# InSilicoModellingGroup/rdcFEs

Hardware: AMD Instinct MI355X
Metric: elements_assembled_per_sec (higher is better)
Workload: dtype f64; 1 GPU; PIHNA TET4 K(119): 10110954 tets, 1728000 nodes, 5 unknowns, params run/PIHNA/input.dat (shipped), order=lex, state of SURVEY App. C (background (0,0,0,7170,0) of the shipped field file, tumour values inside a sphere r = 0.25; see state_sensitivity); scatter=rowgather, kernel_variant=auto, parallelism=single GPU, rank0_local_elements=10110954, rank0_nnz=639395950

## Files before the change

### rdcfes_amd/csrc/rdc_prep.h

```cpp
#ifndef RDC_PREP_H
#define RDC_PREP_H
#include <stdint.h>
#include <string>
#include <vector>

namespace rdc {

struct HostPrep {
  int nen = 0, nvar = 0;
  int64_t n_elem = 0, n_node = 0, n_owned = 0;
  std::vector<int64_t> bptr;
  std::vector<int32_t> bcol;
  std::vector<uint16_t> eslot;
  int n_colours = 0;
  std::vector<int32_t> colour;
  std::vector<uint32_t> elem_order;
  std::vector<int64_t> colour_ptr;
  std::vector<uint64_t> first_mask;
  std::vector<uint8_t> first_rhs;
  bool rowgather_ok = false;
  int rg_block = 256;
  size_t rg_lds_bytes = 0;
  std::vector<uint32_t> pair_elem;
  std::vector<uint8_t> pair_local;
// ... 49 lines not shown

struct SolidGather {
  std::vector<uint32_t> gptr, gsrc;
  std::vector<int32_t> brow;
};
std::string solid_gather_build(const HostPrep& P, SolidGather& out);

struct HostPrepEv {
  static constexpr int MAXN = 16, NBP = 256, BLOCK = 256;
  struct Desc {
    uint32_t nown, nvis, ntouch, nb;
    uint32_t out_doubles;
    uint32_t min_node, max_node, pad;
  };
  struct Node {
    uint32_t bptr;
    uint16_t len, blk0;
    uint32_t obase;
    uint32_t node;
  };
  bool ok = false;
  int nls = 0;
  size_t max_out_doubles = 0;
  std::vector<Desc> desc;
  std::vector<uint32_t> nlist;
  std::vector<uint32_t> vloc;
  std::vector<uint32_t> vslot;
  std::vector<Node> ntab;
  std::vector<uint8_t> bpart;
  int64_t n_visits = 0, n_rows = 0;
  int64_t n_conflicts = 0;
  int64_t n_group_rows = 0;
  int64_t n_pass_instr = 0;
  static constexpr int PASS_COST_PIHNA[4] = {69, 54, 39, 24};
  static constexpr int PASS_COST_FLAT[4] = {40, 40, 40, 40};
  static constexpr int COLLISION_COST = 17;
};
std::string prep_build_ev(const HostPrep& P, const uint32_t* conn, size_t lds_budget_bytes, HostPrepEv& out, int64_t n_interior = -1);

#if defined(__HIPCC__)
#define RDC_EVL __host__ __device__ inline __attribute__((always_inline))
#else
#define RDC_EVL inline
#endif
namespace evl {
constexpr uint32_t IDLE = 0xFFFFFFFFu;
RDC_EVL uint32_t vloc_pack(const uint32_t (&pos)[4]) { return pos[0] | pos[1] << 8 | pos[2] << 16 | pos[3] << 24; }
RDC_EVL int vloc_pos(uint32_t pl, int j) { return (int)((pl >> (8 * j)) & 0xFF); }
RDC_EVL int vloc_rows(const int (&li)[4], int nown) { return (li[0] < nown) + (li[1] < nown) + (li[2] < nown) + (li[3] < nown); }
RDC_EVL void vslot_add(uint32_t (&sl)[2], int i, int j, uint32_t slot) { sl[i >> 1] |= (slot & 15u) << (16 * (i & 1) + 4 * j); }
RDC_EVL int vslot_get(uint32_t w0, uint32_t w1, int i, int j) { return (int)(((i < 2 ? w0 : w1) >> (16 * (i & 1) + 4 * j)) & 0xF); }
RDC_EVL int block(int a, int s) { return s * HostPrepEv::MAXN + a; }
RDC_EVL int block_node(int t) { return t & (HostPrepEv::MAXN - 1); }
RDC_EVL int block_slot(int t) { return t >> 4; }
RDC_EVL int seg_entry(int nv, int len, int a, int s, int b) { return a * (nv * len) + nv * s + b; }
RDC_EVL int seg_phase(uint32_t obase) { return (int)(obase & 1u); }
}

struct HostPrepCl {
  struct Limits { int max_nodes = 24, max_pairs = 192, max_elems = 64, max_row_doubles = 6000, pair_order = 1, img_per_block = 0; };
  struct Desc {
    uint16_t nown, npair, nelem, pad;
    uint32_t row_doubles;
    uint32_t min_node_max_node_pad;
  };
  struct Node {
// ... 75 lines not shown
```

### rdcfes_amd/csrc/rdc_prep_ev.cpp

```cpp
#include <algorithm>
#include <array>
#include <cstring>
#include <numeric>

#include "rdc_prep.h"

namespace rdc {

std::string prep_build_ev(const HostPrep& P, const uint32_t* conn, size_t lds_budget_bytes, HostPrepEv& E, int64_t n_interior) {
  E = HostPrepEv();
  if (P.nen != 4 || (P.nvar != 5 && P.nvar != 3)) return "element-visit lists exist for TET4 with 3 or 5 unknowns only";
  const size_t nv2 = (size_t)P.nvar * P.nvar;
  const int64_t n_elem = P.n_elem, n_node = P.n_node, n_owned = P.n_owned;
  if (n_owned <= 0) return "no owned nodes";
  if (P.bptr[(size_t)n_owned] >= ((int64_t)1 << 32)) return "more than 2^32 node blocks";
  constexpr int MAXN = HostPrepEv::MAXN, NBP = HostPrepEv::NBP, BLOCK = HostPrepEv::BLOCK;
  std::vector<int64_t> inc_ptr((size_t)n_node + 1, 0);
  for (int64_t x = 0; x < n_elem * 4; x++) inc_ptr[conn[x] + 1]++;
  for (int64_t n = 0; n < n_node; n++) inc_ptr[n + 1] += inc_ptr[n];
  std::vector<uint32_t> inc((size_t)inc_ptr[n_node]);
  {
    std::vector<int64_t> fill(inc_ptr.begin(), inc_ptr.end() - 1);
    for (int64_t e = 0; e < n_elem; e++)
      for (int i = 0; i < 4; i++) inc[fill[conn[e * 4 + i]]++] = (uint32_t)e;
  }
  const size_t budget_doubles = lds_budget_bytes / sizeof(double);
  std::vector<int32_t> cluster_of((size_t)n_owned, -1);
  std::vector<std::vector<uint32_t>> clusters;
  {
    std::vector<uint32_t> emark((size_t)n_elem, 0), nmark((size_t)n_node, 0), gain((size_t)n_owned, 0), gstamp((size_t)n_owned, 0);
    uint32_t stamp = 0;
    std::vector<uint32_t> cand, tmp, rejected;
    std::vector<int32_t> free_nb((size_t)n_owned, 0);
    int max_nb = 0;
    for (int64_t n = 0; n < n_owned; n++) {
      if (P.bptr[n + 1] - P.bptr[n] > NBP / MAXN) return "a node has more than 16 node blocks in its row (valence > 15): no element-visit lists";
      int c = 0;
      for (int64_t b = P.bptr[n]; b < P.bptr[n + 1]; b++) c += (P.bcol[b] != (int32_t)n && (int64_t)P.bcol[b] < n_owned);
// ... 97 lines not shown
#pragma omp parallel for schedule(dynamic, 256)
  for (int64_t w = 0; w < nwg; w++) {
    const std::vector<uint32_t>& cl = clusters[(size_t)w];
    std::vector<uint32_t>& vis = visits[(size_t)w];
    for (uint32_t n : cl)
      for (int64_t k = inc_ptr[n]; k < inc_ptr[n + 1]; k++) vis.push_back(inc[k]);
    std::sort(vis.begin(), vis.end());
    vis.erase(std::unique(vis.begin(), vis.end()), vis.end());
    std::vector<uint32_t>& t = touched[(size_t)w];
    for (uint32_t e : vis)
      for (int j = 0; j < 4; j++) t.push_back(conn[(int64_t)e * 4 + j]);
    std::sort(t.begin(), t.end());
    t.erase(std::unique(t.begin(), t.end()), t.end());
    std::vector<uint32_t> ordered(cl.begin(), cl.end());
    for (uint32_t m : t) if (!((int64_t)m < n_owned && cluster_of[m] == (int32_t)w)) ordered.push_back(m);
    t.swap(ordered);
    ntouch_w[(size_t)w] = (int32_t)t.size();
    if (t.size() > 255 || vis.size() > (size_t)BLOCK) {
#pragma omp atomic write
      fail = 1;
    }
  }
  if (fail) return "internal: cluster limits violated";
  int mx = 1;
  for (int64_t w = 0; w < nwg; w++) mx = std::max(mx, (int)ntouch_w[(size_t)w]);
  E.nls = (mx + 63) & ~63;
  E.nlist.assign((size_t)nwg * E.nls, 0);
  E.vloc.assign((size_t)nwg * BLOCK, 0xFFFFFFFFu);
  E.vslot.assign((size_t)nwg * BLOCK * 2, 0);
  E.ntab.assign((size_t)nwg * MAXN, HostPrepEv::Node{0, 0, 0, 0, 0});
  E.bpart.assign((size_t)nwg * NBP, 0);
  std::vector<int64_t> rows_w((size_t)nwg, 0), conf_w((size_t)nwg, 0), pass_w((size_t)nwg, 0), instr_w((size_t)nwg, 0);
  std::vector<size_t> img_w((size_t)nwg, 0);
#pragma omp parallel for schedule(dynamic, 256)
  for (int64_t w = 0; w < nwg; w++) {
    const std::vector<uint32_t>& cl = clusters[(size_t)w];
    const std::vector<uint32_t>& t = touched[(size_t)w];
    const std::vector<uint32_t>& vis = visits[(size_t)w];
    HostPrepEv::Desc& d = E.desc[(size_t)w];
    bool wfail = false;
    d.nown = (uint32_t)cl.size(); d.nvis = (uint32_t)vis.size(); d.ntouch = (uint32_t)t.size(); d.pad = 0;
    d.min_node = *std::min_element(cl.begin(), cl.end());
    d.max_node = *std::max_element(cl.begin(), cl.end());
    uint32_t* nl = &E.nlist[(size_t)w * E.nls];
    for (int x = 0; x < E.nls; x++) nl[x] = t[std::min<size_t>((size_t)x, t.size() - 1)];
    uint32_t blk = 0, ob = 0;
    for (size_t x = 0; x < cl.size(); x++) {
      const uint32_t n = cl[x];
      HostPrepEv::Node& nd = E.ntab[(size_t)w * MAXN + x];
      const int64_t len = P.bptr[n + 1] - P.bptr[n];
      nd.bptr = (uint32_t)P.bptr[n]; nd.len = (uint16_t)len; nd.blk0 = (uint16_t)x; nd.node = n;
      const uint32_t phase = (uint32_t)(((int64_t)nv2 * P.bptr[n]) & 1);
      if ((uint32_t)evl::seg_phase(ob) != phase) ob++;
      nd.obase = ob;
      ob += (uint32_t)(nv2 * (size_t)len);
      blk += (uint32_t)len;
      if (len > NBP / MAXN) wfail = true;
    }
    d.nb = blk;
    if (wfail) {
#pragma omp atomic write
      fail = 1;
      continue;
    }
    {
      uint8_t* bp = &E.bpart[(size_t)w * NBP];
// ... 179 lines not shown
        try_profile(prof, best_pl);
      }
    }
    if (!best_pl.ok) wfail = true;
    std::vector<int> fill_g(16, 0), maxr_g(16, 0);
    for (int x = 0; x < nlanes && !wfail; x++) {
      const V& v = vv[(size_t)x];
      const int best_g = best_pl.grp[(size_t)x];
      const int* pm = PERM4[PERM_R[v.r][(int)best_pl.q[(size_t)x]]];
      int perm[4];
      for (int i = 0; i < v.r; i++) perm[i] = v.own[pm[i]];
      for (int j = v.r; j < 4; j++) perm[j] = v.rest[j - v.r];
      maxr_g[best_g] = std::max(maxr_g[best_g], v.r);
      const size_t lane = (size_t)best_g * 16 + (size_t)fill_g[best_g]++;
      uint32_t li[4];
      for (int j = 0; j < 4; j++) {
        const uint32_t m = conn[(int64_t)v.e * 4 + perm[j]];
        li[j] = (uint32_t)(std::find(t.begin(), t.end(), m) - t.begin());
      }
      E.vloc[(size_t)w * BLOCK + lane] = evl::vloc_pack(li);
      rows_w[(size_t)w] += v.r;
      uint32_t sl2[2] = {0, 0};
      for (int i = 0; i < v.r; i++) {
        for (int j = 0; j < 4; j++) {
          const uint32_t sl = P.eslot[(size_t)v.e * 16 + (size_t)perm[i] * 4 + (size_t)perm[j]];
          if (sl > 15) wfail = true;
          evl::vslot_add(sl2, i, j, sl);
        }
        if (li[i] >= cl.size()) wfail = true;
      }
      E.vslot[((size_t)w * BLOCK + lane) * 2] = sl2[0];
      E.vslot[((size_t)w * BLOCK + lane) * 2 + 1] = sl2[1];
    }
    conf_w[(size_t)w] = best_pl.coll;
    instr_w[(size_t)w] = best_pl.instr;
    for (int g = 0; g < 16; g++) pass_w[(size_t)w] += maxr_g[g];
    if (wfail) {
#pragma omp atomic write
      fail = 1;
    }
  }
  if (fail) return "internal: element-visit list construction failed";
  for (int64_t w = 0; w < nwg; w++) {
    E.max_out_doubles = std::max(E.max_out_doubles, img_w[(size_t)w]);
    E.n_visits += (int64_t)E.desc[(size_t)w].nvis;
    E.n_rows += rows_w[(size_t)w];
    E.n_conflicts += conf_w[(size_t)w];
    E.n_group_rows += pass_w[(size_t)w];
    E.n_pass_instr += instr_w[(size_t)w];
  }
  E.ok = true;
  return std::string();
}

}
```

### rdcfes_amd/csrc/rdc_tet4_ev.h

```cpp
#ifndef RDC_TET4_EV_H
#define RDC_TET4_EV_H
#include "rdc_integrands.h"

namespace rdc {
namespace ev {

constexpr int NM = 16;
constexpr int NMG = 22;
constexpr int NBP = 256;
constexpr int MAXN = 16;
enum { M_E1, M_EoV, M_EPh, M_EQh, M_En, M_Ec, M_Eh, M_Ev, M_Ea, M_Ex, M_Ey, M_ETau, M_EdTc, M_Epv, M_Eg4, M_Edd,
       M_Xc, M_Yc, M_Zc, M_Xh, M_Yh, M_Zh };
constexpr bool symmetric_moment(int m) { return m != M_Epv; }
constexpr bool symmetric_moment_gen(int m) { return m != M_Epv && m != M_Edd && m != M_Xc && m != M_Yc && m != M_Xh && m != M_Yh; }

template <int EXP_MODE, class Sink, bool MIRROR = true, bool GEN = false>
RDC_HD void pihna_visit(const PihnaK& k, const double (&X)[4][3], const double (&U)[4][5], const int r, Sink& sink, const bool bg = false) {
  double e1[3], e2[3], e3[3];
#pragma unroll
  for (int d = 0; d < 3; d++) { e1[d] = X[1][d] - X[0][d]; e2[d] = X[2][d] - X[0][d]; e3[d] = X[3][d] - X[0][d]; }
  double g[4][3];
  g[1][0] = e2[1] * e3[2] - e2[2] * e3[1]; g[1][1] = e2[2] * e3[0] - e2[0] * e3[2]; g[1][2] = e2[0] * e3[1] - e2[1] * e3[0];
  g[2][0] = e3[1] * e1[2] - e3[2] * e1[1]; g[2][1] = e3[2] * e1[0] - e3[0] * e1[2]; g[2][2] = e3[0] * e1[1] - e3[1] * e1[0];
  g[3][0] = e1[1] * e2[2] - e1[2] * e2[1]; g[3][1] = e1[2] * e2[0] - e1[0] * e2[2]; g[3][2] = e1[0] * e2[1] - e1[1] * e2[0];
  const double det = e1[0] * g[1][0] + e1[1] * g[1][1] + e1[2] * g[1][2];
  const double inv = rcp(det), inv2 = inv * inv;
  const double adet = fabs(det);
#pragma unroll
  for (int d = 0; d < 3; d++) g[0][d] = -(g[1][d] + g[2][d] + g[3][d]);
  const double Wc = adet * (-2.0 / 15.0), Wh = adet * 0.075;
  const double a0 = Wc * (1.0 / 16.0), b36 = Wh * (1.0 / 36.0), w18 = Wh * (1.0 / 18.0);
  Pihna::Pt s[5];
  {
    double S[5];
#pragma unroll
    for (int v = 0; v < 5; v++) S[v] = (U[0][v] + U[1][v]) + (U[2][v] + U[3][v]);
#pragma unroll
    for (int q = 0; q < 5; q++) {
      double uq[5];
#pragma unroll
      for (int v = 0; v < 5; v++) uq[v] = (q == 0) ? 0.25 * S[v] : (S[v] * (1.0 / 6.0) + U[q == 0 ? 0 : q - 1][v] * (1.0 / 3.0));
      Pihna::point<EXP_MODE>(k, uq, nullptr, s[q]);
    }
  }
#define RDC_EV_SYM(m, beta)                                                                              \
  {                                                                                                      \
    const double Sm_ = a0 * beta[0] + b36 * ((beta[1] + beta[2]) + (beta[3] + beta[4]));                 \
    const double t_[4] = {w18 * beta[1], w18 * beta[2], w18 * beta[3], w18 * beta[4]};                   \
// ... 109 lines not shown
        RDC_EV_PT(b, ((sp == 1 ? s[q].c : s[q].h) > k.Lambda) ? (expr) : 0.0)                             \
        FSx = (scale) * (Wc * 0.25 * b[0] + Wh * (1.0 / 6.0) * ((b[1] + b[2]) + (b[3] + b[4])));         \
        _Pragma("unroll") for (int j = 0; j < 4; j++) fx[j] = (scale) * (Wh * (1.0 / 3.0)) * b[j + 1];   \
      }
      RDC_EV_F(FS1, f1, Td, s[q].dT)
      RDC_EV_F(FS2, f2, Tt, s[q].dT * (sp == 1 ? s[q].c : s[q].h))
      RDC_EV_F(FS3, f3, Tt, s[q].Tau)
#undef RDC_EV_F
      {
        RDC_EV_PT(b, ((sp == 1 ? s[q].c : s[q].h) > k.Lambda) ? s[q].Tau : 0.0)
        sD = Td * (Wc * b[0] + Wh * ((b[1] + b[2]) + (b[3] + b[4])));
      }
      {
        RDC_EV_PT(b, ((sp == 1 ? s[q].c : s[q].h) > k.Lambda) ? s[q].Tau * (sp == 1 ? s[q].c : s[q].h) : 0.0)
        sZ = Tt * (Wc * b[0] + Wh * ((b[1] + b[2]) + (b[3] + b[4])));
      }
      const int mX = sp == 1 ? M_Xc : M_Xh, mY = sp == 1 ? M_Yc : M_Yh, mZ = sp == 1 ? M_Zc : M_Zh;
#pragma unroll
      for (int i = 0; i < 4; i++) if (i < r) {
        const double gko = go[0] * g[i][0] + go[1] * g[i][1] + go[2] * g[i][2];
        const double gkv = gv[0] * g[i][0] + gv[1] * g[i][1] + gv[2] * g[i][2];
        const double xb = gko * FS1 + gkv * FS2, yb = gkv * FS3;
#pragma unroll
        for (int j = 0; j < 4; j++) {
          const double dd_ = g[i][0] * g[j][0] + g[i][1] * g[j][1] + g[i][2] * g[j][2];
          sink.mom(mX, i, j, xb + gko * f1[j] + gkv * f2[j]);
          sink.mom(mY, i, j, yb + gkv * f3[j] + sD * dd_);
          if (!MIRROR || j >= i) sink.mom(mZ, i, j, sZ * dd_);
        }
        sink.rhs(sp, i, -(sD * gko + sZ * gkv));
      }
    }
  }
  if (!bg) {
    RDC_EV_PT(oneVe, 1.0 - s[q].Ve)
    RDC_EV_PT(Pq, s[q].Ve * s[q].rV)
    RDC_EV_PT(Qq, oneVe[q] * s[q].rV)
    RDC_EV_SYM(M_EoV, oneVe)
    {
      RDC_EV_PT(Ph, Pq[q] * s[q].h)
      RDC_EV_SYM(M_EPh, Ph)
      RDC_EV_PT(xx, k.Tc2h * (Pq[q] * s[q].c) + k.Th2c * Ph[q])
      RDC_EV_SYM(M_Ex, xx)
    }
    {
      RDC_EV_PT(Qh, Qq[q] * s[q].h)
      RDC_EV_SYM(M_EQh, Qh)
      RDC_EV_PT(yy, k.Tc2h * (Qq[q] * s[q].c) + k.Th2c * Qh[q])
      RDC_EV_SYM(M_Ey, yy)
    }
    {
      RDC_EV_PT(G, s[q].n + k.Tn_c * (s[q].c * s[q].n) + k.Tn_h * (s[q].h * s[q].n) + k.Tn_v * (s[q].v * s[q].n) + k.Th2n * (oneVe[q] * s[q].h))
      RDC_EV_RHS(0, G)
    }
    {
      RDC_EV_PT(G, s[q].c + k.Tprod_c * (s[q].Tau * s[q].c) - k.Tc2h * (oneVe[q] * s[q].c) + k.Th2c * (s[q].h - oneVe[q] * s[q].h) - k.Tn_c * (s[q].c * s[q].n))
      RDC_EV_RHS(1, G)
    }
    {
      RDC_EV_PT(G, s[q].h + k.Tc2h * (oneVe[q] * s[q].c) - k.Th2c * (s[q].h - oneVe[q] * s[q].h) - k.Tn_h * (s[q].h * s[q].n) - k.Th2n * (oneVe[q] * s[q].h))
      RDC_EV_RHS(2, G)
    }
  }
  if (!bg) {
    RDC_EV_PT(G, s[q].a + k.Tsec_c * s[q].c + k.Tsec_h * s[q].h - k.Tupt * (s[q].v * s[q].a) - k.Tdec * s[q].a)
    RDC_EV_RHS(4, G)
  }
#undef RDC_EV_RHS
  {
    const double one[5] = {1.0, 1.0, 1.0, 1.0, 1.0};
    RDC_EV_SYM(M_E1, one)
  }
  if (!bg) {
    { RDC_EV_PT(b, s[q].n) RDC_EV_SYM(M_En, b) }
    { RDC_EV_PT(b, s[q].c) RDC_EV_SYM(M_Ec, b) }
    { RDC_EV_PT(b, s[q].h) RDC_EV_SYM(M_Eh, b) }
    { RDC_EV_PT(b, s[q].dT * s[q].c) RDC_EV_SYM(M_EdTc, b) }
  }
  { RDC_EV_PT(b, s[q].v) RDC_EV_SYM(M_Ev, b) }
  if (k.Tupt != 0.0) { RDC_EV_PT(b, s[q].a) RDC_EV_SYM(M_Ea, b) }
  { RDC_EV_PT(b, s[q].Tau) RDC_EV_SYM(M_ETau, b) }
#undef RDC_EV_SYM
#undef RDC_EV_PT
}

RDC_HD bool pihna_background(const double (&U)[4][5]) {
  bool b = true;
#pragma unroll
  for (int j = 0; j < 4; j++) b = b && U[j][0] == 0.0 && U[j][1] == 0.0 && U[j][2] == 0.0 && U[j][4] == 0.0 && U[j][3] > 0.0;
  return b;
}

template <int NMT>
RDC_HD void pihna_expand(const PihnaK& k, const double (&e)[NMT], double (&o)[25]) {
  const double E1 = e[M_E1], EoV = e[M_EoV], EPh = e[M_EPh], EQh = e[M_EQh], En = e[M_En], Ec = e[M_Ec], Eh = e[M_Eh], Ev = e[M_Ev];
  const double x = e[M_Ex], y = e[M_Ey], pcj = k.Tprod_c * e[M_EdTc], pv = e[M_Epv];
  o[0] = E1 - k.Tn_c * Ec - k.Tn_h * Eh - k.Tn_v * Ev;
  o[1] = -(k.Tn_c * En + k.Th2n * EPh);
  o[2] = -(k.Tn_h * En + k.Th2n * EPh + k.Th2n * EoV);
  o[3] = k.Th2n * EQh - k.Tn_v * En;
  o[4] = 0.0;
  o[5] = k.Tn_c * Ec - pcj;
  o[6] = E1 - k.Tprod_c * e[M_ETau] - pcj + k.Tc2h * EoV + x + k.Tn_c * En;
  o[7] = x - pcj - k.Th2c * (E1 - EoV);
  o[8] = -(pcj + y);
// ... 28 lines not shown
```

### rdcfes_amd/csrc/rdc_tet4_ev.hip

```cpp
#include "rdc_internal.h"
#include <type_traits>
#include "rdc_tet4_ev.h"
#include "rdc_ev_phases.h"

namespace rdc {

template <int ABL_>
struct EvSink {
  static constexpr int ABL = ABL_ == 4 ? 0 : ABL_;
  double* p[4][4];
  double* pr[4];
  double sum = 0.0;
  __device__ __forceinline__ void mom(int m, int i, int j, double v) {
    if (ABL == 0) __hip_atomic_fetch_add(p[i][j] + m * ev::NBP, v, __ATOMIC_RELAXED, __HIP_MEMORY_SCOPE_WORKGROUP);
    else if (ABL == 1) p[i][j][m * ev::NBP] = v;
    else sum += v;
  }
  __device__ __forceinline__ void rhs(int a, int i, double v) {
    if (ABL == 0) __hip_atomic_fetch_add(pr[i] + a * ev::MAXN, v, __ATOMIC_RELAXED, __HIP_MEMORY_SCOPE_WORKGROUP);
    else if (ABL == 1) pr[i][a * ev::MAXN] = v;
    else sum += v;
  }
};


namespace {
template <bool GEN, int NM>
__device__ __forceinline__ void ev_read_moments(const double* lds, const int blk, const int mirror, double (&e)[NM]) {
  constexpr auto sym = [](const int m) { return GEN ? ev::symmetric_moment_gen(m) : ev::symmetric_moment(m); };
  constexpr int NS = [=]() { int n = 0; for (int m = 0; m < NM; m++) n += sym(m); return n; }();
#pragma unroll
  for (int m = 0; m < NM; m++) e[m] = lds[m * ev::NBP + blk];
  if (mirror != blk) {
    double t[NS];
#pragma unroll
    for (int m = 0, x = 0; m < NM; m++)
      if (sym(m)) t[x++] = lds[m * ev::NBP + mirror];
    evl::lds_batch();
    evl::lds_land(t);
#pragma unroll
    for (int m = 0, x = 0; m < NM; m++)
      if (sym(m)) e[m] += t[x++];
  }
}
}

template <int EXP_MODE, int MINW, int ABL = 0, bool GEN = false, int NROW = 5>
__global__ void __launch_bounds__(256, MINW)
k_tet4_ev(const HostPrepEv::Desc* __restrict__ desc, const uint32_t* __restrict__ nlist, const uint32_t* __restrict__ vloc,
          const uint32_t* __restrict__ vslot, const HostPrepEv::Node* __restrict__ ntab, const uint8_t* __restrict__ bpart,
          const uint32_t* __restrict__ wg_perm, const PihnaK k, const double* __restrict__ rec, double* __restrict__ val,
          double* __restrict__ rhs, const int nls, const int wg_begin, const int xcd_n, const int stagger,
          long long* __restrict__ stamps, const int bg_skip) {
  static_assert(NROW == 4 || NROW == 5, "all five equation rows, or all but the a row");
  constexpr int BLOCK = 256, NP = 4;
  constexpr bool TL = ABL == 4;
  long long ts[11];
#define RDC_TS(x) if (TL) ts[x] = __builtin_amdgcn_s_memtime()
  RDC_TS(0);
  constexpr int NM = GEN ? ev::NMG : ev::NM, NBP = ev::NBP, MAXN = ev::MAXN;
  extern __shared__ __attribute__((aligned(16))) double lds[];
  __shared__ __attribute__((aligned(16))) HostPrepEv::Node snode[MAXN];
  typedef __attribute__((address_space(3))) void* lds_ptr;
  typedef const __attribute__((address_space(1))) void* glb_ptr;
  if (stagger > 0 && blockIdx.x < 1024u) {
    const unsigned lds_base = __builtin_amdgcn_s_getreg((7 << 11) | 6);
    const uint32_t slot = lds_base == 0 ? 0u : (lds_base < 144u ? 1u : 2u);
    for (uint32_t i = 0; i < slot * (uint32_t)stagger; i++) __builtin_amdgcn_s_sleep(16);
  }
  int wl = (int)blockIdx.x;
  if (xcd_n > 0) {
    const int q = xcd_n >> 3, rem = xcd_n & 7, x = wl & 7;
    wl = x * q + (x < rem ? x : rem) + (wl >> 3);
  }
  int w = wl + wg_begin;
  if (wg_perm) w = (int)wg_perm[w];
  const int tid = threadIdx.x, lane = tid & 63, wv = tid >> 6;
  double* const R = lds + NM * NBP;
  double* const recs = R + 5 * MAXN;
  evl::zero_slice<NM * NBP * 8>(lds, __builtin_amdgcn_readfirstlane(wv));
  if (tid < 5 * MAXN) lds[NM * NBP + tid] = 0.0;
  const int rounds = nls >> 6;
  uint32_t nid = 0;
  if (wv < rounds) nid = nlist[(size_t)w * nls + wv * 64 + lane];
  const uint32_t pl = vloc[(size_t)w * BLOCK + tid];
  const uint2 sl = reinterpret_cast<const uint2*>(vslot)[(size_t)w * BLOCK + tid];
  const HostPrepEv::Desc d = desc[w];
  const int mirror = (int)bpart[(size_t)w * NBP + tid];
  if (tid < MAXN) snode[tid] = ntab[(size_t)w * MAXN + tid];
  if (wv < rounds) {
    const char* src = reinterpret_cast<const char*>(rec) + (size_t)nid * (NP * 16);
#pragma unroll
    for (int p = 0; p < NP; p++)
      __builtin_amdgcn_global_load_lds((glb_ptr)(src + p * 16), (lds_ptr)evl::rec_at(recs, nls, p, wv * 64), 16, 0, 0);
  }
  RDC_TS(1);
  asm volatile("s_waitcnt vmcnt(0)" ::: "memory");
  RDC_TS(2);
  __syncthreads();
  RDC_TS(3);
  if (pl != evl::IDLE) {
    double X[4][3], U[4][5];
    int li[4];
#pragma unroll
    for (int j = 0; j < 4; j++) {
      li[j] = evl::vloc_pos(pl, j);
      double rr[2 * NP];
#pragma unroll
      for (int p = 0; p < NP; p++) {
        const double2 v2 = evl::rec_piece(recs, nls, p, li[j]);
        rr[2 * p] = v2.x; rr[2 * p + 1] = v2.y;
      }
      X[j][0] = rr[0]; X[j][1] = rr[1]; X[j][2] = rr[2];
#pragma unroll
      for (int v = 0; v < 5; v++) U[j][v] = rr[3 + v];
    }
    const int r = evl::vloc_rows(li, (int)d.nown);
    EvSink<ABL> sink;
    evl::aim(sink, lds, R, li, r, sl);
    const bool bg = bg_skip && __builtin_amdgcn_ballot_w64(!ev::pihna_background(U)) == 0;
    if (ABL != 3) ev::pihna_visit<EXP_MODE, EvSink<ABL>, true, GEN>(k, X, U, r, sink, bg);
    if (ABL == 2 && sink.sum == 1.2345e300) rhs[0] = sink.sum;
  }
  if (TL) asm volatile("s_waitcnt lgkmcnt(0)" ::: "memory");
  RDC_TS(4);
  __syncthreads();
  RDC_TS(5);
  double e[NM];
  const int bn = evl::block_node(tid), bs = evl::block_slot(tid);
  const bool has = bn < (int)d.nown && bs < (int)snode[bn < (int)d.nown ? bn : 0].len;
  if (has) ev_read_moments<GEN>(lds, tid, mirror, e);
  if (tid < (int)d.nown * 5) {
    const int n = tid / 5, a = tid - n * 5;
    rhs[(size_t)snode[n].node * 5 + a] = R[a * MAXN + n];
  }
  RDC_TS(6);
  __syncthreads();
  if (has) {
    double o[25];
    ev::pihna_expand(k, e, o);
    const int len = (int)snode[bn].len;
    double* dst = lds + snode[bn].obase + evl::seg_entry(5, len, 0, bs, 0);
#pragma unroll
    for (int a = 0; a < NROW; a++)
#pragma unroll
      for (int b = 0; b < 5; b++) dst[evl::seg_entry(5, len, a, 0, b)] = o[a * 5 + b];
  }
  RDC_TS(7);
  __syncthreads();
  RDC_TS(8);
  {
    const int wvu = __builtin_amdgcn_readfirstlane(wv);
    HostPrepEv::Node nd[4];
    evl::wave_nodes(snode, wvu, nd);
    const HostPrepEv::Node nd01[2] = {nd[0], nd[1]}, nd23[2] = {nd[2], nd[3]};
    const bool on01[2] = {wvu < (int)d.nown, wvu + 4 < (int)d.nown}, on23[2] = {wvu + 8 < (int)d.nown, wvu + 12 < (int)d.nown};
    if (on01[0]) evl::store_segments<25, 2, 5 * NROW>(lds, val, nd01, on01, lane);
    if (on23[0]) evl::store_segments<25, 2, 5 * NROW>(lds, val, nd23, on23, lane);
  }
  if (TL) {
    RDC_TS(9);
    if (stagger == 0) asm volatile("s_waitcnt vmcnt(0)" ::: "memory");
    RDC_TS(10);
    if (lane == 0 && stamps) {
// ... 3 lines not shown
      o[11] = (long long)__builtin_amdgcn_s_getreg((31 << 11) | 4) | ((long long)__builtin_amdgcn_s_getreg((31 << 11) | 20) << 32);
    }
  }
#undef RDC_TS
}


namespace {
__device__ __forceinline__ void evl_dma16(const void* g, const void* lds_base) {
  const uint32_t b = __builtin_amdgcn_readfirstlane((uint32_t)(uintptr_t)lds_base);
  asm volatile("s_mov_b32 m0, %1\n\ts_nop 0\n\tglobal_load_lds_dwordx4 %0, off" ::"v"(g), "s"(b) : "memory", "m0");
}
}
namespace {
struct EvqLists {
  static constexpr int PL = 0, SL = 1024, MISC = SL + 2048, MIRROR = MISC, SNODE = MISC + 256, DESC = MISC + 512, NL = MISC + 544;
  static constexpr int bytes(int nls) { return NL + 2 * nls * 4; }
};
}
template <int EXP_MODE, bool TL, bool GEN = false, int NROW = 5>
__global__ void __launch_bounds__(256, GEN ? 2 : 3)
k_tet4_evq(const HostPrepEv::Desc* __restrict__ desc, const uint32_t* __restrict__ nlist, const uint32_t* __restrict__ vloc,
           const uint32_t* __restrict__ vslot, const HostPrepEv::Node* __restrict__ ntab, const uint8_t* __restrict__ bpart,
           const PihnaK k, const double* __restrict__ rec, double* __restrict__ val, double* __restrict__ rhs, const int nls,
           const int wg_begin, const int wg_count, long long* __restrict__ stamps, const int bg_skip, int* __restrict__ ticket,
           const uint32_t* __restrict__ wg_perm) {
  static_assert(NROW == 4 || NROW == 5, "k_tet4_ev");
  constexpr int BLOCK = 256, NP = 4;
  constexpr int NM = GEN ? ev::NMG : ev::NM, NBP = ev::NBP, MAXN = ev::MAXN;
  extern __shared__ __attribute__((aligned(16))) double lds[];
  __shared__ __attribute__((aligned(16))) HostPrepEv::Node snode[MAXN];
  __shared__ uint8_t smirror[NBP];
  __shared__ int s_nown;
  __shared__ int s_tk[2];
  double* const R = lds + NM * NBP;
  double* const recs = R + 5 * MAXN;
  char* const lists = reinterpret_cast<char*>(recs + (size_t)NP * nls * 2);
  const int rounds = nls >> 6;
  auto lds_barrier = [&]() { asm volatile("s_waitcnt lgkmcnt(0)\n\ts_barrier" ::: "memory"); };
  const int wv = __builtin_amdgcn_readfirstlane((int)(threadIdx.x >> 6));
  constexpr int NONE = 0x7fffffff;
  int c0 = (int)blockIdx.x, c1 = c0 + (int)gridDim.x, c2 = c0 + 2 * (int)gridDim.x;
  auto cluster_of = [&](const int c) -> int { return c < wg_count ? (wg_perm ? (int)wg_perm[wg_begin + c] : wg_begin + c) : -1; };
  int w0c = cluster_of(c0), w1c = cluster_of(c1), w2c = cluster_of(c2);
#define RDC_TS(x) if (TL && stamps && c0 < wg_count && lane == 0) stamps[((int64_t)c0 * 4 + wv) * 12 + x] = __builtin_amdgcn_s_memtime()
  auto fetch = [&](const int w, const uint32_t nid, const int w2, const int nb2, const int lane) {
    if (wv < rounds) {
      const char* src = reinterpret_cast<const char*>(rec) + (size_t)nid * (NP * 16);
#pragma unroll
      for (int p = 0; p < NP; p++) evl_dma16(src + p * 16, evl::rec_at(recs, nls, p, wv * 64));
    }
    if (wv == 0) evl_dma16(reinterpret_cast<const char*>(vloc + (size_t)w * BLOCK) + lane * 16, lists + EvqLists::PL);
    else if (wv < 3) evl_dma16(reinterpret_cast<const char*>(vslot + (size_t)w * BLOCK * 2) + (wv - 1) * 1024 + lane * 16, lists + EvqLists::SL + (wv - 1) * 1024);
    else {
      if (lane < 34) {
        const char* src = lane < 16 ? reinterpret_cast<const char*>(bpart + (size_t)w * NBP) + lane * 16
                        : lane < 32 ? reinterpret_cast<const char*>(ntab + (size_t)w * MAXN) + (lane - 16) * 16
                                    : reinterpret_cast<const char*>(desc + w) + (lane - 32) * 16;
        evl_dma16(src, lists + EvqLists::MISC);
      }
      if (w2 >= 0 && lane < (nls >> 2)) evl_dma16(reinterpret_cast<const char*>(nlist + (size_t)w2 * nls) + lane * 16, lists + EvqLists::NL + nb2 * nls * 4);
    }
  };
  {
    uint32_t nid0 = 0;
    if (wv < rounds) nid0 = nlist[(size_t)w0c * nls + threadIdx.x];
    asm volatile("s_waitcnt vmcnt(0)" : "+v"(nid0)::"memory");
    fetch(w0c, nid0, w1c, 1, (int)(threadIdx.x & 63));
  }
  int tk = NONE;
  bool pending = false;
#pragma unroll 1
  for (int it = 0;; it++) {
    int lane;
    asm volatile("v_mbcnt_lo_u32_b32 %0, -1, 0\n\tv_mbcnt_hi_u32_b32 %0, -1, %0" : "=v"(lane));
    RDC_TS(0);
    evl::zero_slice<NM * NBP * 8>(lds, wv);
    if (wv * 64 + lane < 5 * MAXN) lds[NM * NBP + wv * 64 + lane] = 0.0;
    asm volatile("s_waitcnt vmcnt(0)" : "+v"(tk)::"memory");
    if (pending && wv == 0 && lane == 0) s_tk[0] = tk == NONE ? NONE : 3 * (int)gridDim.x + tk;
    RDC_TS(1);
    lds_barrier();
    RDC_TS(2);
    if (pending) { c2 = __builtin_amdgcn_readfirstlane(s_tk[0]); w2c = cluster_of(c2); }
    if (c0 >= wg_count) break;
    {
      const int tid = wv * 64 + lane;
      const uint32_t pl = *reinterpret_cast<const uint32_t*>(lists + EvqLists::PL + tid * 4);
      const uint2 sl = *reinterpret_cast<const uint2*>(lists + EvqLists::SL + tid * 8);
      const int nown = (int)reinterpret_cast<const HostPrepEv::Desc*>(lists + EvqLists::DESC)->nown;
      {
        const int blk = evl::block(((wv >> 1) << 3) | (lane & 7), ((wv & 1) << 3) | (lane >> 3));
        smirror[blk] = *reinterpret_cast<const uint8_t*>(lists + EvqLists::MIRROR + blk);
        if (tid < MAXN) snode[tid] = *reinterpret_cast<const HostPrepEv::Node*>(lists + EvqLists::SNODE + tid * 16);
        if (tid == 0) s_nown = nown;
      }
      if (pl != evl::IDLE) {
        double X[4][3], U[4][5];
        int li[4];
#pragma unroll
        for (int j = 0; j < 4; j++) {
          li[j] = evl::vloc_pos(pl, j);
          double rr[2 * NP];
#pragma unroll
          for (int p = 0; p < NP; p++) {
            const double2 v2 = evl::rec_piece(recs, nls, p, li[j]);
            rr[2 * p] = v2.x; rr[2 * p + 1] = v2.y;
          }
          X[j][0] = rr[0]; X[j][1] = rr[1]; X[j][2] = rr[2];
#pragma unroll
          for (int v = 0; v < 5; v++) U[j][v] = rr[3 + v];
        }
        const int r = evl::vloc_rows(li, nown);
        EvSink<0> sink;
        evl::aim(sink, lds, R, li, r, sl);
        const bool bg = bg_skip && __builtin_amdgcn_ballot_w64(!ev::pihna_background(U)) == 0;
        ev::pihna_visit<EXP_MODE, EvSink<0>, true, GEN>(k, X, U, r, sink, bg);
      }
    }
    RDC_TS(3);
    lds_barrier();
    RDC_TS(4);
    asm volatile("v_mbcnt_lo_u32_b32 %0, -1, 0\n\tv_mbcnt_hi_u32_b32 %0, -1, %0" : "=v"(lane));
    const int bn = ((wv >> 1) << 3) | (lane & 7), bs = ((wv & 1) << 3) | (lane >> 3), blk = evl::block(bn, bs);
    int nown = s_nown, mirror = (int)smirror[blk];
    uint32_t bn_len = reinterpret_cast<const uint32_t*>(snode + bn)[1], bn_obase = snode[bn].obase;
    uint32_t base8 = snode[8].obase;
    uint32_t nid = 0;
    if (c1 < wg_count && wv < rounds) nid = *reinterpret_cast<const uint32_t*>(lists + EvqLists::NL + (((it + 1) & 1) * nls + wv * 64 + lane) * 4);
    evl::lds_batch();
    evl::lds_land(nown, mirror); evl::lds_land(bn_len, bn_obase); evl::lds_land(base8, nid);
    nown = __builtin_amdgcn_readfirstlane(nown);
    base8 = __builtin_amdgcn_readfirstlane(base8);
    bn_len &= 0xFFFFu;
    if (c1 < wg_count) fetch(w1c, nid, w2c, it & 1, lane);
    tk = NONE;
    if (c2 < wg_count && wv == 0 && lane == 0) {
      const int one = 1;
      asm volatile("global_atomic_add %0, %1, %2, off sc0" : "=v"(tk) : "v"(ticket), "v"(one) : "memory");
    }
    pending = true;
    double e[NM];
    const bool has = bn < nown && bs < (int)bn_len;
#pragma unroll
    for (int m = 0; m < NM; m++) e[m] = 0.0;
    if (has) ev_read_moments<GEN>(lds, blk, mirror, e);
    {
      const int tid = wv * 64 + lane;
      if (tid < nown * 5) {
        const int n = tid / 5, a = tid - n * 5;
        rhs[(size_t)snode[n].node * 5 + a] = R[a * MAXN + n];
      }
    }
    double o[25];
    ev::pihna_expand(k, e, o);
    lds_barrier();
#pragma unroll 1
    for (int h = 0; h < 2; h++) {
      const int n0 = h * 8;
      if (n0 >= nown) break;
      const uint32_t base = h == 0 ? 0u : (base8 & ~1u);
      if ((wv >> 1) == h && has) {
        const int len = (int)bn_len;
        double* dst = lds + (bn_obase - base) + evl::seg_entry(5, len, 0, bs, 0);
#pragma unroll
        for (int a = 0; a < NROW; a++)
#pragma unroll
          for (int b = 0; b < 5; b++) dst[evl::seg_entry(5, len, a, 0, b)] = o[a * 5 + b];
      }
      evl::v4u_t raw[2];
      evl::wave_nodes_read(snode, n0 + wv, raw);
      HostPrepEv::Node ndh[2];
      evl::wave_nodes_land(raw, ndh);
      lds_barrier();
      const int n1 = nown < n0 + 8 ? nown : n0 + 8;
      const bool on[2] = {n0 + wv < n1, n0 + wv + 4 < n1};
      if (on[0]) evl::store_segments<25, 2, 5 * NROW>(lds, val, ndh, on, lane, base);
      lds_barrier();
    }
// ... 66 lines not shown
```

Measured before the change: 7.488 billion elements/s.

## Skip dead moment LDS reads for all-background clusters and remap record slots

Each wave writes a per-wave background flag to LDS. When all four waves in a cluster visited only background elements, the moment read stage loads only the moments a background visit can produce and zeros the rest. This cuts LDS reads and mirror adds. Host prep also adds an LDS bank-conflict model and reassigns non-owned record slots (a remap of vloc and nlist) to reduce conflicts on 128-bit record reads. The cost is extra branching and templated read variants, and the remap changes ntouch and could mis-map slots if it is wrong.

```diff
diff --git a/rdcfes_amd/csrc/rdc_lds_model.h b/rdcfes_amd/csrc/rdc_lds_model.h
--- /dev/null
+++ b/rdcfes_amd/csrc/rdc_lds_model.h
@@ -0,0 +1,117 @@
+#ifndef RDC_LDS_MODEL_H
+#define RDC_LDS_MODEL_H
+#include <cstdint>
+
+#include "rdc_prep.h"
+
+namespace rdc {
+namespace ldsm {
+
+inline int group_b128(const int lane) {
+  const int l = lane & 31;
+  const bool first = l < 4 || (l >= 12 && l < 16) || (l >= 20 && l < 28);
+  return 2 * (lane >> 5) + (first ? 0 : 1);
+}
+inline int group_b64(const int lane) { return lane >> 4; }
+
+inline int group_cycles(const uint32_t* addr, const int n, const int width) {
+  uint32_t seen[16][16];
+  int cnt[16] = {0};
+  int worst = 0;
+  for (int x = 0; x < n; x++) {
+    const int s = (int)((addr[x] / (uint32_t)width) & 15u);
+    bool dup = false;
+    for (int y = 0; y < cnt[s] && !dup; y++) dup = seen[s][y] == addr[x];
+    if (!dup && cnt[s] < 16) seen[s][cnt[s]++] = addr[x];
+    if (cnt[s] > worst) worst = cnt[s];
+  }
+  return worst;
+}
+
+struct Cycles {
+  int64_t ideal = 0, cycles = 0;
+  Cycles& operator+=(const Cycles& o) { ideal += o.ideal; cycles += o.cycles; return *this; }
+};
+
+template <class Group>
+inline Cycles wave_cycles(const uint32_t (&addr)[64], const bool (&active)[64], const int width, Group group) {
+  uint32_t a[4][16];
+  int n[4] = {0, 0, 0, 0};
+  for (int lane = 0; lane < 64; lane++)
+    if (active[lane]) { const int g = group(lane); if (n[g] < 16) a[g][n[g]++] = addr[lane]; }
+  Cycles c;
+  for (int g = 0; g < 4; g++) { c.ideal += n[g] > 0; c.cycles += group_cycles(a[g], n[g], width); }
+  return c;
+}
+
+
+inline Cycles record_reads(const uint32_t* vloc, const int pieces, const uint8_t* remap = nullptr) {
+  Cycles c;
+  for (int wv = 0; wv < 4; wv++)
+    for (int j = 0; j < 4; j++) {
+      uint32_t addr[64];
+      bool active[64];
+      for (int lane = 0; lane < 64; lane++) {
+        const uint32_t pl = vloc[wv * 64 + lane];
+        active[lane] = pl != evl::IDLE;
+        const int pos = evl::vloc_pos(pl, j);
+        addr[lane] = active[lane] ? 16u * (uint32_t)(remap ? remap[pos] : pos) : 0u;
+      }
+      const Cycles one = wave_cycles(addr, active, 16, group_b128);
+      c.ideal += pieces * one.ideal;
+      c.cycles += pieces * one.cycles;
+    }
+  return c;
+}
+
+enum Mapping { MAP_EV = 0, MAP_EVQ = 1 };
+inline int lane_block(const Mapping map, const int wv, const int lane) {
+  if (map == MAP_EV) return wv * 64 + lane;
+  return evl::block(((wv >> 1) << 3) | (lane & 7), ((wv & 1) << 3) | (lane >> 3));
+}
+inline bool lane_has(const HostPrepEv::Desc& d, const HostPrepEv::Node* ntab, const int blk) {
+  const int bn = evl::block_node(blk), bs = evl::block_slot(blk);
+  return bn < (int)d.nown && bs < (int)ntab[bn].len;
+}
+
+inline void moment_reads(const HostPrepEv::Desc& d, const HostPrepEv::Node* ntab, const uint8_t* bpart, const Mapping map, Cycles& own, Cycles& mirror) {
+  for (int wv = 0; wv < 4; wv++) {
+    uint32_t a_own[64], a_mir[64];
+    bool on_own[64], on_mir[64];
+    for (int lane = 0; lane < 64; lane++) {
+      const int blk = lane_block(map, wv, lane);
+      on_own[lane] = lane_has(d, ntab, blk);
+      on_mir[lane] = on_own[lane] && (int)bpart[blk] != blk;
+      a_own[lane] = 8u * (uint32_t)blk;
+      a_mir[lane] = 8u * (uint32_t)bpart[blk];
+    }
+    own += wave_cycles(a_own, on_own, 8, group_b64);
+    mirror += wave_cycles(a_mir, on_mir, 8, group_b64);
+  }
+}
+
+inline Cycles image_writes(const HostPrepEv::Desc& d, const HostPrepEv::Node* ntab, const Mapping map, const int nrow) {
+  Cycles c;
+  const uint32_t base8 = d.nown > 8 ? (ntab[8].obase & ~1u) : 0u;
+  for (int wv = 0; wv < 4; wv++)
+    for (int a = 0; a < nrow; a++)
+      for (int b = 0; b < 5; b++) {
+        uint32_t addr[64];
+        bool active[64];
+        for (int lane = 0; lane < 64; lane++) {
+          const int blk = lane_block(map, wv, lane);
+          active[lane] = lane_has(d, ntab, blk);
+          addr[lane] = 0;
+          if (!active[lane]) continue;
+          const HostPrepEv::Node& nd = ntab[evl::block_node(blk)];
+          const uint32_t base = map == MAP_EVQ && evl::block_node(blk) >= 8 ? base8 : 0u;
+          addr[lane] = 8u * (nd.obase - base + (uint32_t)evl::seg_entry(5, (int)nd.len, a, evl::block_slot(blk), b));
+        }
+        c += wave_cycles(addr, active, 8, group_b64);
+      }
+  return c;
+}
+
+}
+}
+#endif
diff --git a/rdcfes_amd/csrc/rdc_prep.h b/rdcfes_amd/csrc/rdc_prep.h
--- a/rdcfes_amd/csrc/rdc_prep.h
+++ b/rdcfes_amd/csrc/rdc_prep.h
@@ -105,6 +105,9 @@
   int64_t n_conflicts = 0;
   int64_t n_group_rows = 0;
   int64_t n_pass_instr = 0;
+  int64_t lds_rec_ideal = 0, lds_rec = 0, lds_rec_identity = 0;
+  struct LdsExpansion { int64_t own_ideal = 0, own = 0, mirror_ideal = 0, mirror = 0, image_ideal = 0, image = 0; };
+  LdsExpansion lds_exp[2];
   static constexpr int PASS_COST_PIHNA[4] = {69, 54, 39, 24};
   static constexpr int PASS_COST_FLAT[4] = {40, 40, 40, 40};
   static constexpr int COLLISION_COST = 17;
diff --git a/rdcfes_amd/csrc/rdc_prep_ev.cpp b/rdcfes_amd/csrc/rdc_prep_ev.cpp
--- a/rdcfes_amd/csrc/rdc_prep_ev.cpp
+++ b/rdcfes_amd/csrc/rdc_prep_ev.cpp
@@ -4,6 +4,7 @@
 #include <numeric>
 
 #include "rdc_prep.h"
+#include "rdc_lds_model.h"
 
 namespace rdc {
 
@@ -167,6 +168,7 @@
   E.bpart.assign((size_t)nwg * NBP, 0);
   std::vector<int64_t> rows_w((size_t)nwg, 0), conf_w((size_t)nwg, 0), pass_w((size_t)nwg, 0), instr_w((size_t)nwg, 0);
   std::vector<size_t> img_w((size_t)nwg, 0);
+  std::vector<int64_t> rec_w((size_t)nwg, 0), rec_ident_w((size_t)nwg, 0), rec_ideal_w((size_t)nwg, 0), mom_w((size_t)nwg * 12, 0);
 #pragma omp parallel for schedule(dynamic, 256)
   for (int64_t w = 0; w < nwg; w++) {
     const std::vector<uint32_t>& cl = clusters[(size_t)w];
@@ -412,6 +414,97 @@
       E.vslot[((size_t)w * BLOCK + lane) * 2] = sl2[0];
       E.vslot[((size_t)w * BLOCK + lane) * 2 + 1] = sl2[1];
     }
+    if (!wfail) {
+      const int nown = (int)cl.size(), ntouch = (int)t.size(), limit = std::min(E.nls, 255);
+      uint32_t* vl = &E.vloc[(size_t)w * BLOCK];
+      std::array<std::array<uint8_t, 16>, 64> cnt;
+      for (auto& c : cnt) c.fill(0);
+      std::vector<std::vector<uint8_t>> occ((size_t)ntouch);
+      for (int lane = 0; lane < BLOCK; lane++) {
+        if (vl[lane] == evl::IDLE) continue;
+        for (int j = 0; j < 4; j++) {
+          const int g = ((lane >> 6) * 4 + j) * 4 + ldsm::group_b128(lane & 63);
+          std::vector<uint8_t>& o = occ[(size_t)evl::vloc_pos(vl[lane], j)];
+          if (std::find(o.begin(), o.end(), (uint8_t)g) == o.end()) o.push_back((uint8_t)g);
+        }
+      }
+      uint8_t gmax[64];
+      auto regmax = [&](int g) { gmax[g] = *std::max_element(cnt[(size_t)g].begin(), cnt[(size_t)g].end()); };
+      for (int p = 0; p < nown; p++) for (uint8_t g : occ[(size_t)p]) cnt[g][(size_t)(p & 15)]++;
+      for (int g = 0; g < 64; g++) regmax(g);
+      int room[16];
+      for (int r = 0; r < 16; r++) { room[r] = 0; for (int p = r; p < limit; p += 16) room[r] += p >= nown; }
+      std::vector<int8_t> res((size_t)ntouch, -1);
+      auto added = [&](int p, int r) { int c = 0; for (uint8_t g : occ[(size_t)p]) c += cnt[g][(size_t)r] + 1 > gmax[g]; return c; };
+      auto place = [&](int p, int r) { for (uint8_t g : occ[(size_t)p]) if (++cnt[g][(size_t)r] > gmax[g]) gmax[g] = cnt[g][(size_t)r]; room[r]--; res[(size_t)p] = (int8_t)r; };
+      auto lift = [&](int p) { const int r = res[(size_t)p]; for (uint8_t g : occ[(size_t)p]) { cnt[g][(size_t)r]--; regmax(g); } room[r]++; res[(size_t)p] = -1; };
+      auto best_of = [&](int p, int keep) {
+        int br = -1, bc = 0;
+        for (int r = 0; r < 16; r++) {
+          if (room[r] <= 0) continue;
+          const int c = added(p, r);
+          if (br < 0 || c < bc || (c == bc && br != keep && (r == keep || room[r] > room[br]))) { br = r; bc = c; }
+        }
+        return br;
+      };
+      std::vector<int> order;
+      for (int p = nown; p < ntouch; p++) order.push_back(p);
+      std::stable_sort(order.begin(), order.end(), [&](int a, int b) { return occ[(size_t)a].size() > occ[(size_t)b].size(); });
+      bool placed = true;
+      for (int p : order) { const int r = best_of(p, -1); if (r < 0) { placed = false; break; } place(p, r); }
+      for (int sweep = 0; sweep < 3 && placed; sweep++) {
+        bool moved = false;
+        for (int p : order) {
+          const int r0 = res[(size_t)p];
+          lift(p);
+          const int r = best_of(p, r0);
+          place(p, r);
+          moved = moved || r != r0;
+        }
+        if (!moved) break;
+      }
+      const ldsm::Cycles before = ldsm::record_reads(vl, 1);
+      rec_ident_w[(size_t)w] = before.cycles;
+      rec_ideal_w[(size_t)w] = before.ideal;
+      rec_w[(size_t)w] = before.cycles;
+      if (placed) {
+        uint8_t remap[256];
+        for (int p = 0; p < 256; p++) remap[p] = (uint8_t)p;
+        int next[16];
+        for (int r = 0; r < 16; r++) { next[r] = r; while (next[r] < nown) next[r] += 16; }
+        int top = nown;
+        for (int p = nown; p < ntouch; p++) {
+          const int r = res[(size_t)p];
+          remap[p] = (uint8_t)next[r];
+          next[r] += 16;
+          top = std::max(top, (int)remap[p] + 1);
+        }
+        const ldsm::Cycles after = ldsm::record_reads(vl, 1, remap);
+        if (after.cycles < before.cycles && top <= limit) {
+          for (int lane = 0; lane < BLOCK; lane++) {
+            if (vl[lane] == evl::IDLE) continue;
+            uint32_t li[4];
+            for (int j = 0; j < 4; j++) li[j] = remap[evl::vloc_pos(vl[lane], j)];
+            vl[lane] = evl::vloc_pack(li);
+          }
+          for (int x = 0; x < E.nls; x++) nl[x] = t[0];
+          for (int p = 0; p < ntouch; p++) nl[remap[p]] = t[(size_t)p];
+          d.ntouch = (uint32_t)top;
+          rec_w[(size_t)w] = after.cycles;
+        }
+      }
+      if (P.nvar == 5) {
+        const uint8_t* bp = &E.bpart[(size_t)w * NBP];
+        const HostPrepEv::Node* nt = &E.ntab[(size_t)w * MAXN];
+        for (int map = 0; map < 2; map++) {
+          ldsm::Cycles own, mir;
+          ldsm::moment_reads(d, nt, bp, (ldsm::Mapping)map, own, mir);
+          const ldsm::Cycles img = ldsm::image_writes(d, nt, (ldsm::Mapping)map, 4);
+          int64_t* o = &mom_w[((size_t)w * 2 + (size_t)map) * 6];
+          o[0] = own.ideal; o[1] = own.cycles; o[2] = mir.ideal; o[3] = mir.cycles; o[4] = img.ideal; o[5] = img.cycles;
+        }
+      }
+    }
     conf_w[(size_t)w] = best_pl.coll;
     instr_w[(size_t)w] = best_pl.instr;
     for (int g = 0; g < 16; g++) pass_w[(size_t)w] += maxr_g[g];
@@ -428,6 +521,14 @@
     E.n_conflicts += conf_w[(size_t)w];
     E.n_group_rows += pass_w[(size_t)w];
     E.n_pass_instr += instr_w[(size_t)w];
+    E.lds_rec_ideal += rec_ideal_w[(size_t)w];
+    E.lds_rec_identity += rec_ident_w[(size_t)w];
+    E.lds_rec += rec_w[(size_t)w];
+    for (int map = 0; map < 2; map++) {
+      const int64_t* o = &mom_w[((size_t)w * 2 + (size_t)map) * 6];
+      HostPrepEv::LdsExpansion& x = E.lds_exp[map];
+      x.own_ideal += o[0]; x.own += o[1]; x.mirror_ideal += o[2]; x.mirror += o[3]; x.image_ideal += o[4]; x.image += o[5];
+    }
   }
   E.ok = true;
   return std::string();
diff --git a/rdcfes_amd/csrc/rdc_tet4_ev.h b/rdcfes_amd/csrc/rdc_tet4_ev.h
--- a/rdcfes_amd/csrc/rdc_tet4_ev.h
+++ b/rdcfes_amd/csrc/rdc_tet4_ev.h
@@ -14,6 +14,9 @@
 constexpr bool symmetric_moment(int m) { return m != M_Epv; }
 constexpr bool symmetric_moment_gen(int m) { return m != M_Epv && m != M_Edd && m != M_Xc && m != M_Yc && m != M_Xh && m != M_Yh; }
 
+constexpr bool background_moment(const int m, const bool uptake) {
+  return m == M_E1 || m == M_Ev || m == M_ETau || m == M_Epv || m == M_Edd || m == M_Eg4 || (uptake && m == M_Ea);
+}
 template <int EXP_MODE, class Sink, bool MIRROR = true, bool GEN = false>
 RDC_HD void pihna_visit(const PihnaK& k, const double (&X)[4][3], const double (&U)[4][5], const int r, Sink& sink, const bool bg = false) {
   double e1[3], e2[3], e3[3];
@@ -189,6 +192,8 @@
       }
     }
   }
+  static_assert(!background_moment(M_EoV, true) && !background_moment(M_EPh, true) && !background_moment(M_Ex, true) &&
+                !background_moment(M_EQh, true) && !background_moment(M_Ey, true), "emitted behind !bg");
   if (!bg) {
     RDC_EV_PT(oneVe, 1.0 - s[q].Ve)
     RDC_EV_PT(Pq, s[q].Ve * s[q].rV)
@@ -228,6 +233,12 @@
     const double one[5] = {1.0, 1.0, 1.0, 1.0, 1.0};
     RDC_EV_SYM(M_E1, one)
   }
+  static_assert(!background_moment(M_En, true) && !background_moment(M_Ec, true) && !background_moment(M_Eh, true) &&
+                !background_moment(M_EdTc, true), "emitted behind !bg");
+  static_assert(background_moment(M_E1, false) && background_moment(M_Ev, false) && background_moment(M_ETau, false) &&
+                background_moment(M_Epv, false) && background_moment(M_Edd, false) && background_moment(M_Eg4, false),
+                "emitted whatever bg");
+  static_assert(background_moment(M_Ea, true) && !background_moment(M_Ea, false), "emitted behind k.Tupt != 0 alone");
   if (!bg) {
     { RDC_EV_PT(b, s[q].n) RDC_EV_SYM(M_En, b) }
     { RDC_EV_PT(b, s[q].c) RDC_EV_SYM(M_Ec, b) }
diff --git a/rdcfes_amd/csrc/rdc_tet4_ev.hip b/rdcfes_amd/csrc/rdc_tet4_ev.hip
--- a/rdcfes_amd/csrc/rdc_tet4_ev.hip
+++ b/rdcfes_amd/csrc/rdc_tet4_ev.hip
@@ -25,12 +25,14 @@
 
 
 namespace {
-template <bool GEN, int NM>
-__device__ __forceinline__ void ev_read_moments(const double* lds, const int blk, const int mirror, double (&e)[NM]) {
-  constexpr auto sym = [](const int m) { return GEN ? ev::symmetric_moment_gen(m) : ev::symmetric_moment(m); };
+template <bool GEN, int LIVE, int NM>
+__device__ __forceinline__ void ev_read_moments_of(const double* lds, const int blk, const int mirror, double (&e)[NM]) {
+  static_assert(LIVE == 0 || !GEN, "with every term on, the moments a background visit adds to depend on Lambda");
+  constexpr auto live = [](const int m) { return LIVE == 0 || ev::background_moment(m, LIVE == 2); };
+  constexpr auto sym = [=](const int m) { return live(m) && (GEN ? ev::symmetric_moment_gen(m) : ev::symmetric_moment(m)); };
   constexpr int NS = [=]() { int n = 0; for (int m = 0; m < NM; m++) n += sym(m); return n; }();
 #pragma unroll
-  for (int m = 0; m < NM; m++) e[m] = lds[m * ev::NBP + blk];
+  for (int m = 0; m < NM; m++) e[m] = live(m) ? lds[m * ev::NBP + blk] : 0.0;
   if (mirror != blk) {
     double t[NS];
 #pragma unroll
@@ -42,6 +44,19 @@
     for (int m = 0, x = 0; m < NM; m++)
       if (sym(m)) e[m] += t[x++];
   }
+}
+template <bool GEN, int NM>
+__device__ __forceinline__ void ev_read_moments(const double* lds, const int blk, const int mirror, double (&e)[NM], const bool cluster_bg,
+                                                const bool uptake) {
+  if constexpr (GEN) ev_read_moments_of<GEN, 0>(lds, blk, mirror, e);
+  else if (!cluster_bg) ev_read_moments_of<GEN, 0>(lds, blk, mirror, e);
+  else if (!uptake) ev_read_moments_of<GEN, 1>(lds, blk, mirror, e);
+  else ev_read_moments_of<GEN, 2>(lds, blk, mirror, e);
+}
+constexpr uint32_t EV_ALL_WAVES_BG = 0x01010101u;
+__device__ __forceinline__ void ev_flag_wave(uint8_t* flags, const int wv, const bool bg) {
+  const uint64_t active = __builtin_amdgcn_ballot_w64(true);
+  if (__builtin_amdgcn_mbcnt_hi((uint32_t)(active >> 32), __builtin_amdgcn_mbcnt_lo((uint32_t)active, 0u)) == 0u) flags[wv] = bg ? 1 : 0;
 }
 }
 
@@ -55,12 +70,14 @@
   static_assert(NROW == 4 || NROW == 5, "all five equation rows, or all but the a row");
   constexpr int BLOCK = 256, NP = 4;
   constexpr bool TL = ABL == 4;
+  constexpr bool FLAGS = !GEN && ABL != 3;
   long long ts[11];
 #define RDC_TS(x) if (TL) ts[x] = __builtin_amdgcn_s_memtime()
   RDC_TS(0);
   constexpr int NM = GEN ? ev::NMG : ev::NM, NBP = ev::NBP, MAXN = ev::MAXN;
   extern __shared__ __attribute__((aligned(16))) double lds[];
   __shared__ __attribute__((aligned(16))) HostPrepEv::Node snode[MAXN];
+  __shared__ __attribute__((aligned(4))) uint8_t s_bg[4];
   typedef __attribute__((address_space(3))) void* lds_ptr;
   typedef const __attribute__((address_space(1))) void* glb_ptr;
   if (stagger > 0 && blockIdx.x < 1024u) {
@@ -88,6 +105,7 @@
   const HostPrepEv::Desc d = desc[w];
   const int mirror = (int)bpart[(size_t)w * NBP + tid];
   if (tid < MAXN) snode[tid] = ntab[(size_t)w * MAXN + tid];
+  if (FLAGS && lane == 0) s_bg[wv] = 1;
   if (wv < rounds) {
     const char* src = reinterpret_cast<const char*>(rec) + (size_t)nid * (NP * 16);
 #pragma unroll
@@ -120,6 +138,7 @@
     evl::aim(sink, lds, R, li, r, sl);
     const bool bg = bg_skip && __builtin_amdgcn_ballot_w64(!ev::pihna_background(U)) == 0;
     if (ABL != 3) ev::pihna_visit<EXP_MODE, EvSink<ABL>, true, GEN>(k, X, U, r, sink, bg);
+    if (FLAGS) ev_flag_wave(s_bg, wv, bg);
     if (ABL == 2 && sink.sum == 1.2345e300) rhs[0] = sink.sum;
   }
   if (TL) asm volatile("s_waitcnt lgkmcnt(0)" ::: "memory");
@@ -129,7 +148,8 @@
   double e[NM];
   const int bn = evl::block_node(tid), bs = evl::block_slot(tid);
   const bool has = bn < (int)d.nown && bs < (int)snode[bn < (int)d.nown ? bn : 0].len;
-  if (has) ev_read_moments<GEN>(lds, tid, mirror, e);
+  const bool cluster_bg = FLAGS && __builtin_amdgcn_readfirstlane(*reinterpret_cast<const uint32_t*>(s_bg)) == EV_ALL_WAVES_BG;
+  if (has) ev_read_moments<GEN>(lds, tid, mirror, e, cluster_bg, k.Tupt != 0.0);
   if (tid < (int)d.nown * 5) {
     const int n = tid / 5, a = tid - n * 5;
     rhs[(size_t)snode[n].node * 5 + a] = R[a * MAXN + n];
@@ -199,6 +219,7 @@
   __shared__ __attribute__((aligned(16))) HostPrepEv::Node snode[MAXN];
   __shared__ uint8_t smirror[NBP];
   __shared__ int s_nown;
+  __shared__ __attribute__((aligned(4))) uint8_t s_bg[4];
   __shared__ int s_tk[2];
   double* const R = lds + NM * NBP;
   double* const recs = R + 5 * MAXN;
@@ -261,6 +282,7 @@
         smirror[blk] = *reinterpret_cast<const uint8_t*>(lists + EvqLists::MIRROR + blk);
         if (tid < MAXN) snode[tid] = *reinterpret_cast<const HostPrepEv::Node*>(lists + EvqLists::SNODE + tid * 16);
         if (tid == 0) s_nown = nown;
+        if (!GEN && lane == 0) s_bg[wv] = 1;
       }
       if (pl != evl::IDLE) {
         double X[4][3], U[4][5];
@@ -283,6 +305,7 @@
         evl::aim(sink, lds, R, li, r, sl);
         const bool bg = bg_skip && __builtin_amdgcn_ballot_w64(!ev::pihna_background(U)) == 0;
         ev::pihna_visit<EXP_MODE, EvSink<0>, true, GEN>(k, X, U, r, sink, bg);
+        if (!GEN) ev_flag_wave(s_bg, wv, bg);
       }
     }
     RDC_TS(3);
@@ -293,10 +316,13 @@
     int nown = s_nown, mirror = (int)smirror[blk];
     uint32_t bn_len = reinterpret_cast<const uint32_t*>(snode + bn)[1], bn_obase = snode[bn].obase;
     uint32_t base8 = snode[8].obase;
+    uint32_t wbg = GEN ? 0u : *reinterpret_cast<const uint32_t*>(s_bg);
     uint32_t nid = 0;
     if (c1 < wg_count && wv < rounds) nid = *reinterpret_cast<const uint32_t*>(lists + EvqLists::NL + (((it + 1) & 1) * nls + wv * 64 + lane) * 4);
     evl::lds_batch();
     evl::lds_land(nown, mirror); evl::lds_land(bn_len, bn_obase); evl::lds_land(base8, nid);
+    if (!GEN) evl::lds_land(wbg);
+    const bool cluster_bg = !GEN && __builtin_amdgcn_readfirstlane(wbg) == EV_ALL_WAVES_BG;
     nown = __builtin_amdgcn_readfirstlane(nown);
     base8 = __builtin_amdgcn_readfirstlane(base8);
     bn_len &= 0xFFFFu;
@@ -311,7 +337,9 @@
     const bool has = bn < nown && bs < (int)bn_len;
 #pragma unroll
     for (int m = 0; m < NM; m++) e[m] = 0.0;
-    if (has) ev_read_moments<GEN>(lds, blk, mirror, e);
+    double tupt = k.Tupt;
+    asm volatile("" : "+s"(tupt));
+    if (has) ev_read_moments<GEN>(lds, blk, mirror, e, cluster_bg, tupt != 0.0);
     {
       const int tid = wv * 64 + lane;
       if (tid < nown * 5) {
```

Result: no change. 7.508 billion elements/s, median of 3 (+0.3%).
